# liortalker/MindTheEdge

Measured on NVIDIA B200. Metric: edge_loss_fwd_bwd_throughput, higher is better.
Workload: dtype f32

## Files before the change

### mindtheedge_b200/csrc/common.cuh

```cuda
#pragma once
#include <cuda_runtime.h>
#include <stdint.h>
#include <stdlib.h>

#include <mutex>
#include <utility>
#include <vector>

#include "../../include/mte.h"

#define MTE_FULL_MASK 0xffffffffu

#define MTE_RETURN_IF_CUDA_ERROR()                        \
    do {                                                  \
        cudaError_t e__ = cudaGetLastError();             \
        if (e__ != cudaSuccess) return (int)e__;          \
    } while (0)

namespace mte {

struct DevInfo {
    int sms;
    int smemOptin;
};
inline int current_device() {
    int d = 0;
    cudaGetDevice(&d);
    return d;
}
inline DevInfo dev_info() {
    constexpr int kMaxDev = 64;
    static DevInfo cache[kMaxDev];
    static bool have[kMaxDev];
    static std::mutex mu;
    const int d = current_device();
    std::lock_guard<std::mutex> lock(mu);
    if (d >= 0 && d < kMaxDev && have[d]) return cache[d];
    DevInfo v{148, 232448};
    cudaDeviceGetAttribute(&v.sms, cudaDevAttrMultiProcessorCount, d);
    cudaDeviceGetAttribute(&v.smemOptin, cudaDevAttrMaxSharedMemoryPerBlockOptin, d);
    if (v.sms < 1) v.sms = 1;
    if (d >= 0 && d < kMaxDev) { cache[d] = v; have[d] = true; }
    return v;
}
inline int num_sms() { return dev_info().sms; }

inline cudaError_t opt_in_smem(const void *func, int bytes) {
    static std::mutex mu;
    static std::vector<std::pair<const void *, long long>> done;
    const int d = current_device();
    std::lock_guard<std::mutex> lock(mu);
    for (auto &e : done)
        if (e.first == func && (int)(e.second >> 32) == d) {
            if ((int)(e.second & 0xffffffffLL) >= bytes) return cudaSuccess;
            const cudaError_t r = cudaFuncSetAttribute(func, cudaFuncAttributeMaxDynamicSharedMemorySize, bytes);
            if (r == cudaSuccess) e.second = ((long long)d << 32) | (unsigned)bytes;
            return r;
        }
    const cudaError_t r = cudaFuncSetAttribute(func, cudaFuncAttributeMaxDynamicSharedMemorySize, bytes);
    if (r == cudaSuccess) done.emplace_back(func, ((long long)d << 32) | (unsigned)bytes);
    return r;
}

#ifdef MTE_DEBUG_KNOBS
inline const char *debug_knob(const char *name) { return getenv(name); }
#else
inline const char *debug_knob(const char *) { return nullptr; }
#endif

struct WsHeader {
    unsigned int ticket[16];
    unsigned int flag[16];
    unsigned int pad[32];
};
static_assert(sizeof(WsHeader) == 256, "workspace header layout");
constexpr size_t kWsAccumOffset = 4096;
constexpr int kWsMaxLossImages = (MTE_WS_HEADER_BYTES - 4096) / 64;

__host__ __device__ inline size_t align_up(size_t v, size_t a) { return (v + a - 1) / a * a; }
__host__ __device__ inline int ceil_div(int a, int b) { return (a + b - 1) / b; }

__device__ __forceinline__ float warp_sum(float v) {
#pragma unroll
    for (int o = 16; o > 0; o >>= 1) v += __shfl_xor_sync(MTE_FULL_MASK, v, o);
    return v;
}
__device__ __forceinline__ double warp_sum(double v) {
#pragma unroll
    for (int o = 16; o > 0; o >>= 1) v += __shfl_xor_sync(MTE_FULL_MASK, v, o);
    return v;
}
__device__ __forceinline__ unsigned warp_or(unsigned v) {
#pragma unroll
    for (int o = 16; o > 0; o >>= 1) v |= __shfl_xor_sync(MTE_FULL_MASK, v, o);
    return v;
}

__device__ __forceinline__ float4 ld_stream4(const float *p) { return __ldcs(reinterpret_cast<const float4 *>(p)); }
__device__ __forceinline__ float4 ld_cached4(const float *p) { return __ldg(reinterpret_cast<const float4 *>(p)); }
__device__ __forceinline__ void st_stream4(float *p, float4 v) { __stcs(reinterpret_cast<float4 *>(p), v); }

inline bool aligned16(const void *p) { return (reinterpret_cast<uintptr_t>(p) & 15u) == 0; }

namespace canny {
int run_level_hysteresis(const unsigned char *cl, unsigned char *E, int N, int H, int W, int T, void *scratch,
                         cudaStream_t st);
size_t hysteresis_scratch_bytes(int N, int H, int W);
}

}
```

### mindtheedge_b200/csrc/edge_loss_fused.cu

```cuda
#include <string.h>

#include "edge_loss_kernels.cuh"

namespace mte {
namespace loss {

#ifndef MTE_FUSED_D
#define MTE_FUSED_D 3
#endif
constexpr int kFusedD = MTE_FUSED_D;
#ifndef MTE_FUSED_SEGCOST
#define MTE_FUSED_SEGCOST 2
#endif
constexpr int kSegCostFused = MTE_FUSED_SEGCOST;
#ifndef MTE_FUSED_REGS
#define MTE_FUSED_REGS 120
#endif
#ifndef MTE_FUSED_P1ROWS
#define MTE_FUSED_P1ROWS 16
#endif
constexpr int kP1Rows = MTE_FUSED_P1ROWS;
__host__ __device__ constexpr int fused_smem_bytes() { return kRWarps * kFusedD * 3 * 512; }

__device__ __forceinline__ unsigned ld_acquire_u32(const unsigned *p) {
    unsigned v;
    asm volatile("ld.acquire.gpu.global.u32 %0, [%1];" : "=r"(v) : "l"(p) : "memory");
    return v;
}

__device__ __forceinline__ void grid_barrier(unsigned *ctr, unsigned nCtas) {
    __syncthreads();
    if (threadIdx.x == 0) {
        __threadfence();
        atomicAdd(ctr, 1u);
#ifdef MTE_FUSED_NOSLEEP
        while (ld_acquire_u32(ctr) < nCtas) {}
#else
        while (ld_acquire_u32(ctr) < nCtas) __nanosleep(20);
#endif
        __threadfence();
    }
    __syncthreads();
}

#ifdef MTE_FUSED_TRACE
__device__ __forceinline__ unsigned long long gtime() {
    unsigned long long t;
    asm volatile("mov.u64 %0, %globaltimer;" : "=l"(t));
    return t;
}
#define MTE_TRACE(slot, isMin)                                                                                   \
    do {                                                                                                         \
        __syncthreads();                                                                                         \
        if (threadIdx.x == 0) {                                                                                  \
            const unsigned long long t_ = gtime();                                                               \
            atomicMax(reinterpret_cast<unsigned long long *>(F.barrier) + 128 + (slot), (isMin) ? ~t_ : t_); \
        }                                                                                                        \
    } while (0)
#else
#define MTE_TRACE(slot, isMin) do {} while (0)
#endif

struct FusedP {
    LossP L;
    const float *expectG;
    unsigned *barrier;
};

struct Seg {
    int si, img, strip, row0, nrows;
};
__device__ __forceinline__ bool next_segment(const LossP &P, int &u0, int u1, Seg &s) {
    int si = 0;
#pragma unroll
    for (int k = 1; k < MTE_MAX_SCALES; k++)
        if (k < P.nScales && u0 >= P.s[k].unitBase) si = k;
    const ScaleP &S = P.s[si];
    const int local = u0 - S.unitBase;
    const int HV = ((S.H + 1) >> 1) + kSegCostFused;
    const int t = local / HV;
    const int r = local - t * HV;
    const int take = min(HV - r, u1 - u0);
    s.row0 = 2 * max(r - kSegCostFused, 0);
    s.nrows = min(2 * max(r + take - kSegCostFused, 0), S.H) - s.row0;
    u0 += take;
    s.si = si;
    s.img = t / S.strips;
    s.strip = t - s.img * S.strips;
    return s.nrows > 0;
}

__device__ __forceinline__ void red_add4(float *p, float4 v) {
    asm volatile("red.global.add.v4.f32 [%0], {%1, %2, %3, %4};" ::"l"(p), "f"(v.x), "f"(v.y), "f"(v.z), "f"(v.w) : "memory");
}

__device__ __forceinline__ float2 f2(float s) { return make_float2(s, s); }
__device__ __forceinline__ float2 f2add(float2 a, float2 b) { return __fadd2_rn(a, b); }
__device__ __forceinline__ float2 f2mul(float2 a, float2 b) { return __fmul2_rn(a, b); }
__device__ __forceinline__ float2 f2fma(float2 a, float2 b, float2 c) { return __ffma2_rn(a, b, c); }
__device__ __forceinline__ float2 f2sub(float2 a, float2 b) { return __ffma2_rn(b, f2(-1.f), a); }
__device__ __forceinline__ float2 rcp_rn_normal2(float2 d) {
    float2 r = make_float2(rcp_approx(d.x), rcp_approx(d.y));
    const float2 nd = f2mul(d, f2(-1.f));
    float2 e = f2fma(nd, r, f2(1.f));
    r = f2fma(r, e, r);
    e = f2fma(nd, r, f2(1.f));
    return f2fma(r, e, r);
}

struct PRow2 {
    float2 c[2], s3[2], d[2];
};
__device__ __forceinline__ void prep_row2(PRow2 &R, const float2 (&x)[2]) {
    const float l = __shfl_up_sync(MTE_FULL_MASK, x[1].y, 1);
    const float r = __shfl_down_sync(MTE_FULL_MASK, x[0].x, 1);
    R.c[0] = x[0];
    R.c[1] = x[1];
    R.s3[0] = make_float2((l + x[0].x) + x[0].y, (x[0].x + x[0].y) + x[1].x);
    R.s3[1] = make_float2((x[0].y + x[1].x) + x[1].y, (x[1].x + x[1].y) + r);
    R.d[0] = make_float2(x[0].y - l, x[1].x - x[0].x);
    R.d[1] = make_float2(x[1].y - x[0].y, r - x[1].x);
}

__device__ __forceinline__ void fused_prologue(const ScaleP &S, const Seg &sg, int lane, unsigned char *ring,
                                               float2 (&xa)[2], float2 (&xc)[2]) {
    constexpr int D = kFusedD;
    constexpr unsigned PLB = 512, SLB = 3 * PLB;
    const int H = S.H, row0 = sg.row0, niter = sg.nrows;
    const unsigned W = (unsigned)S.W;
    const int col0 = (sg.strip * kHaloLanes + lane - 1) * 4;
    const bool colOk = col0 >= 0 && col0 < (int)W;
    const size_t lo = (size_t)sg.img * H * W + (colOk ? col0 : 0);
    const float *xP = S.x + lo, *eP = S.e + lo, *nP = S.n + lo;
    const unsigned ringS = (unsigned)__cvta_generic_to_shared(ring + lane * 16);
    auto load_plain = [&](float2 (&x)[2], int row) {
        x[0] = make_float2(0.f, 0.f);
        x[1] = make_float2(0.f, 0.f);
        if (colOk && row >= 0 && row < H) {
            const float4 t = ld_cached4(elem_addr(xP, (unsigned)row * W));
            x[0] = make_float2(t.x, t.y);
            x[1] = make_float2(t.z, t.w);
        }
    };
    load_plain(xa, row0 - 1);
    load_plain(xc, row0);
#pragma unroll
    for (int k = 0; k < D; k++) {
        if (k < niter) {
            const int rx = row0 + 1 + k;
            cp_async_vec<4>(ringS + k * SLB, elem_addr(xP, (unsigned)min(rx, H - 1) * W), colOk && rx < H);
            const unsigned ro = (unsigned)(row0 + k) * W;
            cp_async_vec<4>(ringS + k * SLB + PLB, elem_addr(eP, ro), colOk);
            cp_async_vec<4>(ringS + k * SLB + 2 * PLB, elem_addr(nP, ro), colOk);
        }
        cp_async_commit();
    }
}

template <bool INV, bool SIG>
__device__ __forceinline__ void fused_segment(const LossP &P, const ScaleP &S, const Seg &sg, int lane,
                                              unsigned char *ring, const float4 *sLut, float cp, float cn,
                                              float2 (&la)[2], float &poison, float2 (&xa)[2], float2 (&xc)[2]) {
    constexpr int D = kFusedD;
    constexpr unsigned PLB = 512, SLB = 3 * PLB;
    constexpr float kFill = INV ? 3.0e38f : 0.f;
    const int H = S.H, row0 = sg.row0, nrows = sg.nrows;
    const unsigned W = (unsigned)S.W;
    const int col0 = (sg.strip * kHaloLanes + lane - 1) * 4;
    const bool colOk = col0 >= 0 && col0 < (int)W;
    const bool writer = colOk && lane >= 1 && lane <= kHaloLanes;
    const size_t lo = (size_t)sg.img * H * W + (colOk ? col0 : 0);
    const float *xP = S.x + lo, *eP = S.e + lo, *nP = S.n + lo;
    float *gP = S.g + lo, *dP = S.dx + lo;
    const bool writeG = writer && S.g != nullptr;
    const float2 mT = f2(-P.T), cp2 = f2(cp), cn2 = f2(cn), eps2 = f2(kEps), one2 = f2(1.f), m1 = f2(-1.f);
    unsigned char *slot0 = ring + lane * 16;
    const unsigned ringS = (unsigned)__cvta_generic_to_shared(slot0);

    auto issue = [&](unsigned so, int j) {
        const int rx = row0 + 1 + j;
        cp_async_vec<4>(ringS + so, elem_addr(xP, (unsigned)min(rx, H - 1) * W), colOk && rx < H);
        const unsigned ro = (unsigned)(row0 + j) * W;
        cp_async_vec<4>(ringS + so + PLB, elem_addr(eP, ro), colOk);
        cp_async_vec<4>(ringS + so + 2 * PLB, elem_addr(nP, ro), colOk);
    };
    auto fix_row = [&](float2 (&x)[2], int row) {
        if (INV) {
            const bool ok = colOk && row >= 0 && row < H;
#pragma unroll
            for (int h = 0; h < 2; h++) {
                const float2 v = make_float2(fmax_nan(ok ? x[h].x : kFill, 1e-6f), fmax_nan(ok ? x[h].y : kFill, 1e-6f));
                x[h] = rcp_rn_normal2(v);
            }
        }
        const float2 t = f2fma(x[0], f2(0.f), f2mul(x[1], f2(0.f)));
        poison += t.x + t.y;
    };
    auto lds2 = [&](float2 (&x)[2], const unsigned char *p) {
        const float4 t = *reinterpret_cast<const float4 *>(p);
        x[0] = make_float2(t.x, t.y);
        x[1] = make_float2(t.z, t.w);
    };

    const int niter = nrows;
    PRow2 win[3];
    fix_row(xa, row0 - 1);
    fix_row(xc, row0);
    prep_row2(win[0], xa);
    prep_row2(win[1], xc);
    float oacc[3][4];
#pragma unroll
    for (int o = 0; o < 3; o++)
#pragma unroll
        for (int v = 0; v < 4; v++) oacc[o][v] = 0.f;
    auto emit = [&](const float (&acc)[4], const PRow2 &dep, int row, bool shared) {
        float out[4];
#pragma unroll
        for (int v = 0; v < 4; v++) {
            float d = acc[v];
            if (INV) {
                const float dp = (v & 1) ? dep.c[v >> 1].y : dep.c[v >> 1].x;
                d = (dp < 1e6f) ? -d * dp * dp : 0.f;
            }
            out[v] = d;
        }
        if (writer) {
            float *o = elem_addr(dP, (unsigned)row * W);
            if (shared) red_add4(o, make_float4(out[0], out[1], out[2], out[3]));
            else st_stream4(o, make_float4(out[0], out[1], out[2], out[3]));
        }
    };

    unsigned so = 0;
#pragma unroll 1
    for (int jj = 0; jj < niter; jj += 3) {
#pragma unroll
        for (int u = 0; u < 3; u++) {
            const int j = jj + u;
            if (j < niter) {
                cp_async_wait<D - 1>();
                float2 xn[2], e[2], th[2];
                lds2(xn, slot0 + so);
                lds2(e, slot0 + so + PLB);
                lds2(th, slot0 + so + 2 * PLB);
                if (j + D < niter) issue(so, j + D);
                cp_async_commit();
                so = (so + SLB == D * SLB) ? 0u : so + SLB;
                const int r = row0 + j;
                PRow2 &dn = win[(u + 2) % 3];
                fix_row(xn, r + 1);
                prep_row2(dn, xn);
                const PRow2 &up = win[u % 3];
                const PRow2 &mid = win[(u + 1) % 3];
                float g[4];
                float2 X[4], Z[4];
#pragma unroll
                for (int h = 0; h < 2; h++) {
                    const float2 Pv = f2sub(dn.s3[h], up.s3[h]);
                    const float2 Dm = mid.d[h];
                    const float2 Rh = f2add(f2add(up.d[h], Dm), dn.d[h]);
                    const float2 dv = f2sub(dn.c[h], up.c[h]);
                    float c0, c1;
                    unsigned cd0, cd1;
                    pick_directional(th[h].x, Pv.x, Rh.x, Dm.x, dv.x, c0, cd0);
                    pick_directional(th[h].y, Pv.y, Rh.y, Dm.y, dv.y, c1, cd1);
                    const float2 gg = make_float2(fabsf(c0), fabsf(c1));
                    g[2 * h] = gg.x;
                    g[2 * h + 1] = gg.y;
                    float2 p = gg;
                    if (SIG) {
                        const float2 nz = f2sub(f2(P.T), gg);
                        p = rcp_rn_normal2(f2add(make_float2(expf(nz.x), expf(nz.y)), one2));
                    }
                    const float2 q = f2fma(p, m1, one2);
                    const float2 pe = f2add(p, eps2), qe = f2add(q, eps2);
                    const float2 ee = e[h], ne = f2fma(ee, m1, one2);
                    la[0] = f2fma(ee, make_float2(lg2_approx(pe.x), lg2_approx(pe.y)), la[0]);
                    la[1] = f2fma(ne, make_float2(lg2_approx(qe.x), lg2_approx(qe.y)), la[1]);
                    float2 d = f2mul(f2mul(cp2, ee), make_float2(rcp_approx(pe.x), rcp_approx(pe.y)));
                    d = f2fma(f2mul(cn2, ne), make_float2(rcp_approx(qe.x), rcp_approx(qe.y)), d);
                    if (SIG) d = f2mul(f2mul(d, p), q);
                    const float d0 = (colOk && gg.x != 0.f) ? d.x : 0.f, d1 = (colOk && gg.y != 0.f) ? d.y : 0.f;
                    const float4 k0 = sLut[cd0 & 15u], k1 = sLut[cd1 & 15u];
                    X[2 * h] = f2mul(f2(d0), make_float2(k0.x, k0.y));
                    Z[2 * h] = f2mul(f2(d0), make_float2(k0.z, k0.w));
                    X[2 * h + 1] = f2mul(f2(d1), make_float2(k1.x, k1.y));
                    Z[2 * h + 1] = f2mul(f2(d1), make_float2(k1.z, k1.w));
                }
                if (writeG) st_stream4(elem_addr(gP, (unsigned)r * W), make_float4(g[0], g[1], g[2], g[3]));
                const float2 Xl = make_float2(__shfl_up_sync(MTE_FULL_MASK, X[3].x, 1), __shfl_up_sync(MTE_FULL_MASK, X[3].y, 1));
                const float2 Xr = make_float2(__shfl_down_sync(MTE_FULL_MASK, X[0].x, 1), __shfl_down_sync(MTE_FULL_MASK, X[0].y, 1));
                const float C2l = __shfl_up_sync(MTE_FULL_MASK, Z[3].y, 1), C2r = __shfl_down_sync(MTE_FULL_MASK, Z[0].y, 1);
#pragma unroll
                for (int v = 0; v < 4; v++) {
                    const float2 xl = v == 0 ? Xl : X[(v + 3) % 4], xr = v == 3 ? Xr : X[(v + 1) % 4];
                    const float c2_l = v == 0 ? C2l : Z[(v + 3) % 4].y, c2_r = v == 3 ? C2r : Z[(v + 1) % 4].y;
                    const float2 U = f2add(xl, make_float2(xr.x, -xr.y));
                    const float SA = U.x + Z[v].x, DC = U.y;
                    oacc[u][v] = SA + DC;
                    oacc[(u + 2) % 3][v] += c2_l - c2_r;
                    oacc[(u + 1) % 3][v] -= SA - DC;
                }
                if (r >= 1) emit(oacc[(u + 1) % 3], up, r - 1, j < 2);
                if (j == niter - 1) {
                    emit(oacc[(u + 2) % 3], mid, r, true);
                    if (r + 1 < H) emit(oacc[u], dn, r + 1, true);
                }
            }
        }
    }
    cp_async_wait<0>();
    if (!writer) {
        la[0] = f2(0.f);
        la[1] = f2(0.f);
    }
}

template <bool INV, bool SIG>
__global__ void __maxnreg__(MTE_FUSED_REGS) edge_loss_fused_kernel(const __grid_constant__ FusedP F) {
    extern __shared__ __align__(16) unsigned char fusedRing[];
    __shared__ float4 sLut[16];
    __shared__ double sLoss[MTE_MAX_SCALES];
    __shared__ int sLast;
    const LossP &P = F.L;
    if (threadIdx.x < 16) {
        const int di = threadIdx.x & 3, sgn_ = threadIdx.x >> 2;
        const float sgn = sgn_ == 1 ? 1.f : (sgn_ == 2 ? -1.f : 0.f);
        const float a = (di == 2 || di == 3) ? 1.f : (di == 1 ? -1.f : 0.f);
        const float c = (di == 2) ? 0.f : 1.f;
        const float bb = (di & 1) ? 1.f : 2.f;
        sLut[threadIdx.x] = make_float4(sgn * a, sgn * c, sgn * a * bb, sgn * c * bb);
    }
    const int lane = threadIdx.x & 31, warp = threadIdx.x >> 5;
    const int nWarps = gridDim.x * kRWarps;
    const int gw = blockIdx.x * kRWarps + warp;
    unsigned char *ring = fusedRing + warp * (fused_smem_bytes() / kRWarps);
    const int uBeg = (int)((long long)P.totalUnits * gw / nWarps);
    const int uEnd = (int)((long long)P.totalUnits * (gw + 1) / nWarps);
    pdl_launch_dependents();
    MTE_TRACE(0, true);
    MTE_TRACE(1, false);

#ifndef MTE_FUSED_TIMING_NO_PHASE1
    {
        int u0 = uBeg;
        while (u0 < uEnd) {
            Seg sg;
            if (!next_segment(P, u0, uEnd, sg)) continue;
            const ScaleP &S = P.s[sg.si];
            const unsigned W = (unsigned)S.W;
            const int col0 = (sg.strip * kHaloLanes + lane - 1) * 4;
            const bool writer = col0 >= 0 && col0 < (int)W && lane >= 1 && lane <= kHaloLanes;
            const float *eP = S.e + (size_t)sg.img * S.H * W + (writer ? col0 : 0);
            if (writer) {
                float *dP = S.dx + (size_t)sg.img * S.H * W + col0;
                const float4 z = make_float4(0.f, 0.f, 0.f, 0.f);
                *reinterpret_cast<float4 *>(elem_addr(dP, (unsigned)sg.row0 * W)) = z;
                *reinterpret_cast<float4 *>(elem_addr(dP, (unsigned)(sg.row0 + sg.nrows - 1) * W)) = z;
            }
            float s0 = 0.f, s1 = 0.f;
#pragma unroll 1
            for (int j0 = 0; j0 < sg.nrows; j0 += kP1Rows) {
                float4 t[kP1Rows];
#pragma unroll
                for (int k = 0; k < kP1Rows; k++) {
                    t[k] = make_float4(0.f, 0.f, 0.f, 0.f);
                    if (writer && j0 + k < sg.nrows)
                        t[k] = *reinterpret_cast<const float4 *>(elem_addr(eP, (unsigned)(sg.row0 + j0 + k) * W));
                }
#pragma unroll
                for (int k = 0; k < kP1Rows; k += 2) {
                    s0 += (t[k].x + t[k].y) + (t[k].z + t[k].w);
                    s1 += (t[k + 1].x + t[k + 1].y) + (t[k + 1].z + t[k + 1].w);
                }
            }
            const float v = warp_sum(s0 + s1);
            unsigned long long *acc = P.accum + (size_t)(S.imgBase + sg.img) * kAcc;
            if (lane == 0) {
                atomicAdd(acc + A_WP, (unsigned long long)__double2ll_rn((double)v * kFix));
                if (!isfinite(v)) atomicOr(acc + A_FLAGS, (unsigned long long)F_NONFINITE);
            }
        }
    }
    int u0 = uBeg;
    Seg sg;
    bool have = false;
    while (u0 < uEnd && !have) have = next_segment(P, u0, uEnd, sg);
    float2 xa[2], xc[2];
    if (have) fused_prologue(P.s[sg.si], sg, lane, ring, xa, xc);
    MTE_TRACE(2, true);
    MTE_TRACE(3, false);
    grid_barrier(F.barrier, gridDim.x);
    MTE_TRACE(4, false);
#else
    __syncthreads();
    int u0 = uBeg;
    Seg sg;
    bool have = false;
    while (u0 < uEnd && !have) have = next_segment(P, u0, uEnd, sg);
    float2 xa[2], xc[2];
    if (have) fused_prologue(P.s[sg.si], sg, lane, ring, xa, xc);
#endif

    while (have) {
        const ScaleP &S = P.s[sg.si];
        const double npix = (double)S.H * (double)S.W;
        float alpha;
        {
            const double wp = (double)(long long)__ldcg(P.accum + (size_t)(S.imgBase + sg.img) * kAcc + A_WP) / kFix;
            const double wn = npix - wp;
            alpha = (float)(wn / (wp + wn));
            if (wn == 0.0) {
                double wnSum = 0.0;
                for (int b = 0; b < S.B; b++)
                    wnSum += npix - (double)(long long)__ldcg(P.accum + (size_t)(S.imgBase + b) * kAcc + A_WP) / kFix;
                if (wnSum == 0.0) alpha = 1.0f;
            }
        }
        float G = F.expectG ? (__ldg(F.expectG) * S.scaleWeight + __ldg(F.expectG + 1 + sg.si)) : S.scaleWeight;
        if (G == 0.f) G = 1.f;
        const float coef = (float)((double)P.weight / (npix * (double)S.B)) * G;
        const float cp = -coef * P.p2n * alpha, cn = coef * (1.0f - alpha);
        float2 la[2] = {make_float2(0.f, 0.f), make_float2(0.f, 0.f)};
        float poison = 0.f;
        fused_segment<INV, SIG>(P, S, sg, lane, ring, sLut, cp, cn, la, poison, xa, xc);
        bool bad = __any_sync(MTE_FULL_MASK, !(poison == 0.f));
        unsigned long long *acc = P.accum + (size_t)(S.imgBase + sg.img) * kAcc;
        const float vp = warp_sum(la[0].x + la[0].y), vn = warp_sum(la[1].x + la[1].y);
        bad = bad || !isfinite(vp) || !isfinite(vn);
        if (lane == 0) {
            atomicAdd(acc + A_SPU, (unsigned long long)__double2ll_rn((double)vp * kFix));
            atomicAdd(acc + A_SNU, (unsigned long long)__double2ll_rn((double)vn * kFix));
            if (bad) atomicOr(acc + A_FLAGS, (unsigned long long)F_NONFINITE);
        }
        have = false;
        while (u0 < uEnd && !have) have = next_segment(P, u0, uEnd, sg);
        if (have) fused_prologue(P.s[sg.si], sg, lane, ring, xa, xc);
    }
    MTE_TRACE(5, true);
    MTE_TRACE(6, false);
    __syncthreads();
    if (threadIdx.x == 0) {
        __threadfence();
        sLast = atomicAdd(P.ticket + 1, 1u) == gridDim.x - 1u;
        __threadfence();
    }
    __syncthreads();
    if (sLast) {
        finalize_loss<false>(P, sLoss);
        __syncthreads();
        if (threadIdx.x == 0) {
            double total = 0.0;
            for (int k = 0; k < P.nScales; k++) {
                total += (double)P.s[k].scaleWeight * sLoss[k];
                float G = F.expectG ? (F.expectG[0] * P.s[k].scaleWeight + F.expectG[1 + k]) : P.s[k].scaleWeight;
                if (G == 0.f) G = 1.f;
                P.ctx[P.totalImages + 2 * MTE_MAX_SCALES + k] = G;
            }
            reinterpret_cast<unsigned *>(P.ctx + P.totalImages + 3 * MTE_MAX_SCALES)[0] = 0u;
            P.lossOut[0] = (float)total;
            P.ticket[0] = 0u;
            P.ticket[1] = 0u;
            *F.barrier = 0u;
        }
        MTE_TRACE(7, false);
    }
}

__global__ void __launch_bounds__(128) edge_loss_rescale_kernel(const __grid_constant__ LossP P, const float *gradLoss,
                                                                float *ctx, float *expectedOut) {
    pdl_wait();
    float *cur = ctx + P.totalImages + 2 * MTE_MAX_SCALES;
    unsigned *done = reinterpret_cast<unsigned *>(ctx + P.totalImages + 3 * MTE_MAX_SCALES);
    bool any = false;
    for (int k = 0; k < P.nScales; k++) any = any || (gradLoss[0] * P.s[k].scaleWeight + gradLoss[1 + k] != cur[k]);
    if (!any) {
        if (expectedOut && blockIdx.x == 0 && threadIdx.x <= P.nScales) expectedOut[threadIdx.x] = gradLoss[threadIdx.x];
        return;
    }
    for (int k = 0; k < P.nScales; k++) {
        const ScaleP &S = P.s[k];
        const float G = gradLoss[0] * S.scaleWeight + gradLoss[1 + k];
        const float c = cur[k];
        if (G == c) continue;
        const float f = G / c;
        const size_t n4 = (size_t)S.B * S.H * S.W / 4;
        float4 *d = reinterpret_cast<float4 *>(S.dx);
        for (size_t i = (size_t)blockIdx.x * blockDim.x + threadIdx.x; i < n4; i += (size_t)gridDim.x * blockDim.x) {
            float4 v = d[i];
            v.x *= f; v.y *= f; v.z *= f; v.w *= f;
            d[i] = v;
        }
    }
    __syncthreads();
    if (threadIdx.x == 0) {
        __threadfence();
        if (atomicAdd(done, 1u) == gridDim.x - 1u) {
            for (int k = 0; k < P.nScales; k++) cur[k] = gradLoss[0] * P.s[k].scaleWeight + gradLoss[1 + k];
            if (expectedOut)
                for (int k = 0; k < 1 + P.nScales; k++) expectedOut[k] = gradLoss[k];
            __threadfence();
            *done = 0u;
        }
    }
}

template <bool INV, bool SIG>
static int launch_fused_one(const FusedP &F, int grid, cudaStream_t st) {
    constexpr int smem = fused_smem_bytes();
    const void *fn = (const void *)edge_loss_fused_kernel<INV, SIG>;
    if (opt_in_smem(fn, smem) != cudaSuccess) return (int)cudaGetLastError();
    int perSm = 0;
    cudaOccupancyMaxActiveBlocksPerMultiprocessor(&perSm, edge_loss_fused_kernel<INV, SIG>, kRThreads, smem);
    if (perSm < 1) return MTE_ERR_ARG;
    const int maxGrid = perSm * num_sms();
    if (grid > maxGrid) grid = maxGrid;
    cudaLaunchConfig_t cfg = {};
    cfg.gridDim = dim3((unsigned)grid);
    cfg.blockDim = dim3((unsigned)kRThreads);
    cfg.dynamicSmemBytes = (size_t)smem;
    cfg.stream = st;
    cudaLaunchAttribute at[1];
    at[0].id = cudaLaunchAttributeCooperative;
    at[0].val.cooperative = 1;
    cfg.attrs = at;
    cfg.numAttrs = 1;
    const cudaError_t e = cudaLaunchKernelEx(&cfg, edge_loss_fused_kernel<INV, SIG>, F);
    return e == cudaSuccess ? MTE_OK : (int)e;
}

int launch_fused(const FusedP &F, int grid, bool inv, bool sig, cudaStream_t st) {
    if (inv) return sig ? launch_fused_one<true, true>(F, grid, st) : launch_fused_one<true, false>(F, grid, st);
    return sig ? launch_fused_one<false, true>(F, grid, st) : launch_fused_one<false, false>(F, grid, st);
}

}
}

using namespace mte;
using namespace mte::loss;

static bool fused_supported(const mte_loss_scale_t *sc, int n, const mte_loss_attrs_t *at) {
    if (!sc || !at || n < 1 || n > MTE_MAX_SCALES) return false;
    if (!at->is_grad) return false;
    for (int i = 0; i < n; i++) {
        const mte_loss_scale_t &s = sc[i];
        if (!s.pred || !s.edge || !s.normal || s.mask) return false;
        if (s.h != s.H || s.w != s.W || s.B < 1 || s.H < 1 || s.W < 4 || (s.W % 4)) return false;
        const void *ptrs[] = {s.pred, s.edge, s.normal, s.grad_map, s.grad_pred};
        for (const void *p : ptrs)
            if (!aligned16(p)) return false;
    }
    return true;
}

extern "C" int mte_edge_loss_fused_supported(const mte_loss_scale_t *sc, int n, const mte_loss_attrs_t *at) {
    return fused_supported(sc, n, at) ? 1 : 0;
}

extern "C" int mte_edge_loss_fwd_grad(const mte_loss_scale_t *sc, int n, const mte_loss_attrs_t *at,
                                      const float *expected_grad_loss, float *loss_out, void *ctx, void *ws,
                                      size_t ws_bytes, mte_stream_t stream) {
    if (!sc || !at || !loss_out || !ctx || !ws) return MTE_ERR_NULL;
    if (!fused_supported(sc, n, at)) return MTE_ERR_ARG;
    for (int i = 0; i < n; i++)
        if (!sc[i].grad_pred) return MTE_ERR_NULL;
    if (ws_bytes < MTE_WS_HEADER_BYTES) return MTE_ERR_WORKSPACE;
    FusedP F;
    memset(&F, 0, sizeof(F));
    LossP &P = F.L;
    int img = 0;
    long long unitBase = 0;
    for (int i = 0; i < n; i++) {
        ScaleP &S = P.s[i];
        S.B = sc[i].B; S.H = sc[i].H; S.W = sc[i].W;
        S.x = sc[i].pred; S.e = sc[i].edge; S.n = sc[i].normal; S.m = nullptr;
        S.g = sc[i].grad_map; S.dx = sc[i].grad_pred; S.stash = nullptr;
        S.strips = ceil_div(S.W, kHaloLanes * 4);
        S.imgBase = img;
        S.unitBase = (int)unitBase;
        unitBase += (long long)S.strips * (((S.H + 1) >> 1) + kSegCostFused) * S.B;
        S.scaleWeight = sc[i].scale_weight;
        img += S.B;
    }
    if (unitBase > 0x7fffffffLL || img > kWsMaxLossImages) return MTE_ERR_SHAPE;
    P.nScales = n; P.totalImages = img; P.totalUnits = (int)unitBase;
    P.T = at->sigmoid_thresh; P.weight = at->weight; P.p2n = at->pos_to_neg;
    char *w = static_cast<char *>(ws);
    WsHeader *hdr = reinterpret_cast<WsHeader *>(w);
    P.accum = reinterpret_cast<unsigned long long *>(w + kWsAccumOffset);
    P.ticket = hdr->ticket;
    P.lossOut = loss_out;
    P.ctx = static_cast<float *>(ctx);
    F.expectG = expected_grad_loss;
    F.barrier = hdr->ticket + 2;
    int grid = num_sms();
    const int minUnits = 2;
    if ((long long)grid * kRWarps * minUnits > unitBase) grid = (int)((unitBase + kRWarps * minUnits - 1) / (kRWarps * minUnits));
    if (grid < 1) grid = 1;
    return launch_fused(F, grid, at->pred_is_inverse != 0, at->is_sigmoid != 0, reinterpret_cast<cudaStream_t>(stream));
}

extern "C" int mte_edge_loss_grad_rescale(const mte_loss_scale_t *sc, int n, const float *grad_loss, void *ctx,
                                          float *expected_out, mte_stream_t stream) {
    if (!sc || !grad_loss || !ctx) return MTE_ERR_NULL;
    if (n < 1 || n > MTE_MAX_SCALES) return MTE_ERR_ARG;
    LossP P;
    memset(&P, 0, sizeof(P));
    int img = 0;
    for (int i = 0; i < n; i++) {
        if (!sc[i].grad_pred) return MTE_ERR_NULL;
        if (!aligned16(sc[i].grad_pred) || (sc[i].W % 4)) return MTE_ERR_ALIGN;
        P.s[i].B = sc[i].B; P.s[i].H = sc[i].H; P.s[i].W = sc[i].W;
        P.s[i].dx = sc[i].grad_pred;
        P.s[i].scaleWeight = sc[i].scale_weight;
        img += sc[i].B;
    }
    P.nScales = n; P.totalImages = img;
    cudaLaunchConfig_t cfg = {};
    cfg.gridDim = dim3((unsigned)num_sms() * 2u);
    cfg.blockDim = dim3(128u);
    cfg.stream = reinterpret_cast<cudaStream_t>(stream);
    cudaLaunchAttribute at[1];
    at[0].id = cudaLaunchAttributeProgrammaticStreamSerialization;
    at[0].val.programmaticStreamSerializationAllowed = 1;
    cfg.attrs = at;
    cfg.numAttrs = 1;
    const cudaError_t e = cudaLaunchKernelEx(&cfg, edge_loss_rescale_kernel, P, grad_loss, static_cast<float *>(ctx), expected_out);
    return e == cudaSuccess ? MTE_OK : (int)e;
}
```

Before: 132,600.

## Split fused loss phase-1 sums into PDL-chained kernel, drop grid barrier

The per-image edge sums that used to be computed in a first phase of the cooperative fused kernel, followed by a software grid barrier, now run in a separate kernel. That kernel streams rows through a cp.async ring buffer in shared memory. The fused kernel is launched with programmatic dependent launch so it can run its prologue while the sums kernel finishes, then calls pdl_wait before the main loop. The aim is to remove the grid-wide spin barrier and cooperative launch and to overlap the prologue with the reduction. It also sets a max-shared carveout and halves the rescale kernel grid, at the cost of one extra kernel launch.

```diff
diff --git a/mindtheedge_b200/csrc/common.cuh b/mindtheedge_b200/csrc/common.cuh
--- a/mindtheedge_b200/csrc/common.cuh
+++ b/mindtheedge_b200/csrc/common.cuh
@@ -45,7 +45,7 @@
 }
 inline int num_sms() { return dev_info().sms; }
 
-inline cudaError_t opt_in_smem(const void *func, int bytes) {
+inline cudaError_t opt_in_smem(const void *func, int bytes, int carveout = -1) {
     static std::mutex mu;
     static std::vector<std::pair<const void *, long long>> done;
     const int d = current_device();
@@ -57,7 +57,9 @@
             if (r == cudaSuccess) e.second = ((long long)d << 32) | (unsigned)bytes;
             return r;
         }
-    const cudaError_t r = cudaFuncSetAttribute(func, cudaFuncAttributeMaxDynamicSharedMemorySize, bytes);
+    cudaError_t r = cudaFuncSetAttribute(func, cudaFuncAttributeMaxDynamicSharedMemorySize, bytes);
+    if (r == cudaSuccess && carveout >= 0)
+        r = cudaFuncSetAttribute(func, cudaFuncAttributePreferredSharedMemoryCarveout, carveout);
     if (r == cudaSuccess) done.emplace_back(func, ((long long)d << 32) | (unsigned)bytes);
     return r;
 }
diff --git a/mindtheedge_b200/csrc/edge_loss_fused.cu b/mindtheedge_b200/csrc/edge_loss_fused.cu
--- a/mindtheedge_b200/csrc/edge_loss_fused.cu
+++ b/mindtheedge_b200/csrc/edge_loss_fused.cu
@@ -16,32 +16,19 @@
 #ifndef MTE_FUSED_REGS
 #define MTE_FUSED_REGS 120
 #endif
-#ifndef MTE_FUSED_P1ROWS
-#define MTE_FUSED_P1ROWS 16
-#endif
-constexpr int kP1Rows = MTE_FUSED_P1ROWS;
 __host__ __device__ constexpr int fused_smem_bytes() { return kRWarps * kFusedD * 3 * 512; }
 
-__device__ __forceinline__ unsigned ld_acquire_u32(const unsigned *p) {
-    unsigned v;
-    asm volatile("ld.acquire.gpu.global.u32 %0, [%1];" : "=r"(v) : "l"(p) : "memory");
-    return v;
-}
-
-__device__ __forceinline__ void grid_barrier(unsigned *ctr, unsigned nCtas) {
-    __syncthreads();
-    if (threadIdx.x == 0) {
-        __threadfence();
-        atomicAdd(ctr, 1u);
-#ifdef MTE_FUSED_NOSLEEP
-        while (ld_acquire_u32(ctr) < nCtas) {}
-#else
-        while (ld_acquire_u32(ctr) < nCtas) __nanosleep(20);
-#endif
-        __threadfence();
-    }
-    __syncthreads();
-}
+#ifndef MTE_SUMS_WARPS
+#define MTE_SUMS_WARPS 16
+#endif
+#ifndef MTE_SUMS_ROWS
+#define MTE_SUMS_ROWS 4
+#endif
+constexpr int kSumWarps = MTE_SUMS_WARPS, kSumThreads = kSumWarps * 32;
+constexpr int kSumRows = MTE_SUMS_ROWS, kSumStages = 4;
+constexpr unsigned kSumRowBytes = 32 * 16;
+constexpr unsigned kSumStageBytes = kSumRows * kSumRowBytes;
+__host__ __device__ constexpr int sums_smem_bytes() { return kSumWarps * kSumStages * (int)kSumStageBytes; }
 
 #ifdef MTE_FUSED_TRACE
 __device__ __forceinline__ unsigned long long gtime() {
@@ -49,22 +36,22 @@
     asm volatile("mov.u64 %0, %globaltimer;" : "=l"(t));
     return t;
 }
-#define MTE_TRACE(slot, isMin)                                                                                   \
-    do {                                                                                                         \
-        __syncthreads();                                                                                         \
-        if (threadIdx.x == 0) {                                                                                  \
-            const unsigned long long t_ = gtime();                                                               \
-            atomicMax(reinterpret_cast<unsigned long long *>(F.barrier) + 128 + (slot), (isMin) ? ~t_ : t_); \
-        }                                                                                                        \
+__device__ __forceinline__ void trace_put(unsigned *base, int slot, bool isMin, unsigned long long t) {
+    atomicMax(reinterpret_cast<unsigned long long *>(base) + 128 + slot, isMin ? ~t : t);
+}
+#define MTE_TRACE(base, slot, isMin)                                   \
+    do {                                                                 \
+        __syncthreads();                                                 \
+        if (threadIdx.x == 0) trace_put((base), (slot), (isMin), gtime()); \
     } while (0)
 #else
-#define MTE_TRACE(slot, isMin) do {} while (0)
+#define MTE_TRACE(base, slot, isMin) do {} while (0)
 #endif
 
 struct FusedP {
     LossP L;
     const float *expectG;
-    unsigned *barrier;
+    unsigned *trace;
 };
 
 struct Seg {
@@ -92,6 +79,109 @@
 
 __device__ __forceinline__ void red_add4(float *p, float4 v) {
     asm volatile("red.global.add.v4.f32 [%0], {%1, %2, %3, %4};" ::"l"(p), "f"(v.x), "f"(v.y), "f"(v.z), "f"(v.w) : "memory");
+}
+
+__device__ __forceinline__ float4 lds_f4(unsigned addr) {
+    float4 v;
+    asm volatile("ld.shared.v4.f32 {%0, %1, %2, %3}, [%4];" : "=f"(v.x), "=f"(v.y), "=f"(v.z), "=f"(v.w) : "r"(addr) : "memory");
+    return v;
+}
+
+__global__ void __launch_bounds__(kSumThreads, 65536 / (kSumThreads * 32)) edge_loss_sums_kernel(const __grid_constant__ FusedP F, int nItems) {
+    extern __shared__ __align__(16) unsigned char sumRing[];
+    __shared__ unsigned sDesc[kSumWarps][kSumStages];
+    const LossP &P = F.L;
+    const int lane = threadIdx.x & 31, warp = threadIdx.x >> 5;
+    const unsigned ringS = (unsigned)__cvta_generic_to_shared(sumRing + warp * kSumStages * kSumStageBytes) + lane * 16;
+    pdl_wait();
+    pdl_launch_dependents();
+    MTE_TRACE(F.trace, 0, true);
+    MTE_TRACE(F.trace, 1, false);
+
+    const int nW = gridDim.x * kSumWarps, gw = blockIdx.x * kSumWarps + warp;
+    int it = (int)((long long)nItems * gw / nW);
+    const int itEnd = (int)((long long)nItems * (gw + 1) / nW);
+    int u0 = 0, u1 = 0, siStrip = 0, img = 0, row = 0, rowEnd = 0;
+    auto produce = [&](int slot) -> bool {
+        while (row >= rowEnd) {
+            if (u0 < u1) {
+                Seg sg;
+                if (next_segment(P, u0, u1, sg)) {
+                    siStrip = sg.si | sg.strip << 2;
+                    img = sg.img;
+                    row = sg.row0;
+                    rowEnd = sg.row0 + sg.nrows;
+                    const ScaleP &S = P.s[sg.si];
+                    const int col0 = (sg.strip * kHaloLanes + lane - 1) * 4;
+                    if (lane >= 1 && lane <= kHaloLanes && col0 < S.W) {
+                        float *dP = S.dx + (size_t)img * S.H * S.W + col0;
+                        const float4 z = make_float4(0.f, 0.f, 0.f, 0.f);
+                        *reinterpret_cast<float4 *>(elem_addr(dP, (unsigned)row * S.W)) = z;
+                        *reinterpret_cast<float4 *>(elem_addr(dP, (unsigned)(rowEnd - 1) * S.W)) = z;
+                    }
+                }
+                continue;
+            }
+            if (it >= itEnd) return false;
+            u0 = (int)((long long)P.totalUnits * it / nItems);
+            u1 = (int)((long long)P.totalUnits * (it + 1) / nItems);
+            it++;
+        }
+        const ScaleP &S = P.s[siStrip & 3];
+        const int strip = siStrip >> 2;
+        const int n = min(kSumRows, rowEnd - row);
+        const int col0 = (strip * kHaloLanes + lane - 1) * 4;
+        const bool ok = lane >= 1 && lane <= kHaloLanes && col0 < S.W;
+        if (lane == 0) sDesc[warp][slot] = (unsigned)(S.imgBase + img) | (unsigned)n << 12 | (row + n == rowEnd ? 1u << 24 : 0u);
+        const float *eP = S.e + (size_t)img * S.H * S.W + (ok ? col0 : 0);
+#pragma unroll
+        for (int k = 0; k < kSumRows; k++)
+            if (k < n) cp_async_vec<4>(ringS + slot * kSumStageBytes + k * kSumRowBytes, elem_addr(eP, (unsigned)(row + k) * S.W), ok);
+        cp_async_commit();
+        row += n;
+        return true;
+    };
+
+    bool more = true;
+    int c = 0, p = 0;
+    for (int k = 0; k < kSumStages && more; k++) {
+        more = produce(k);
+        if (more) p++;
+    }
+    float s0 = 0.f, s1 = 0.f;
+    while (c < p) {
+        const int slot = c & (kSumStages - 1);
+        if (p - c == kSumStages) cp_async_wait<kSumStages - 1>();
+        else cp_async_wait<0>();
+        __syncwarp();
+        const unsigned d = sDesc[warp][slot];
+        const int n = (d >> 12) & 31;
+#pragma unroll
+        for (int k = 0; k < kSumRows; k++) {
+            float4 a = make_float4(0.f, 0.f, 0.f, 0.f);
+            if (k < n) a = lds_f4(ringS + slot * kSumStageBytes + k * kSumRowBytes);
+            if (k & 1) s1 += (a.x + a.y) + (a.z + a.w);
+            else s0 += (a.x + a.y) + (a.z + a.w);
+        }
+        if (d >> 24) {
+            const float v = warp_sum(s0 + s1);
+            if (lane == 0) {
+                unsigned long long *acc = P.accum + (size_t)(d & 0xfffu) * kAcc;
+                atomicAdd(acc + A_WP, (unsigned long long)__double2ll_rn((double)v * kFix));
+                if (!isfinite(v)) atomicOr(acc + A_FLAGS, (unsigned long long)F_NONFINITE);
+            }
+            s0 = 0.f;
+            s1 = 0.f;
+        }
+        __syncwarp();
+        c++;
+        if (more) {
+            more = produce(p & (kSumStages - 1));
+            if (more) p++;
+        }
+    }
+    MTE_TRACE(F.trace, 2, true);
+    MTE_TRACE(F.trace, 3, false);
 }
 
 __device__ __forceinline__ float2 f2(float s) { return make_float2(s, s); }
@@ -331,6 +421,9 @@
         const float bb = (di & 1) ? 1.f : 2.f;
         sLut[threadIdx.x] = make_float4(sgn * a, sgn * c, sgn * a * bb, sgn * c * bb);
     }
+#ifdef MTE_FUSED_TRACE
+    const unsigned long long tStart = gtime();
+#endif
     const int lane = threadIdx.x & 31, warp = threadIdx.x >> 5;
     const int nWarps = gridDim.x * kRWarps;
     const int gw = blockIdx.x * kRWarps + warp;
@@ -338,69 +431,23 @@
     const int uBeg = (int)((long long)P.totalUnits * gw / nWarps);
     const int uEnd = (int)((long long)P.totalUnits * (gw + 1) / nWarps);
     pdl_launch_dependents();
-    MTE_TRACE(0, true);
-    MTE_TRACE(1, false);
-
-#ifndef MTE_FUSED_TIMING_NO_PHASE1
-    {
-        int u0 = uBeg;
-        while (u0 < uEnd) {
-            Seg sg;
-            if (!next_segment(P, u0, uEnd, sg)) continue;
-            const ScaleP &S = P.s[sg.si];
-            const unsigned W = (unsigned)S.W;
-            const int col0 = (sg.strip * kHaloLanes + lane - 1) * 4;
-            const bool writer = col0 >= 0 && col0 < (int)W && lane >= 1 && lane <= kHaloLanes;
-            const float *eP = S.e + (size_t)sg.img * S.H * W + (writer ? col0 : 0);
-            if (writer) {
-                float *dP = S.dx + (size_t)sg.img * S.H * W + col0;
-                const float4 z = make_float4(0.f, 0.f, 0.f, 0.f);
-                *reinterpret_cast<float4 *>(elem_addr(dP, (unsigned)sg.row0 * W)) = z;
-                *reinterpret_cast<float4 *>(elem_addr(dP, (unsigned)(sg.row0 + sg.nrows - 1) * W)) = z;
-            }
-            float s0 = 0.f, s1 = 0.f;
-#pragma unroll 1
-            for (int j0 = 0; j0 < sg.nrows; j0 += kP1Rows) {
-                float4 t[kP1Rows];
-#pragma unroll
-                for (int k = 0; k < kP1Rows; k++) {
-                    t[k] = make_float4(0.f, 0.f, 0.f, 0.f);
-                    if (writer && j0 + k < sg.nrows)
-                        t[k] = *reinterpret_cast<const float4 *>(elem_addr(eP, (unsigned)(sg.row0 + j0 + k) * W));
-                }
-#pragma unroll
-                for (int k = 0; k < kP1Rows; k += 2) {
-                    s0 += (t[k].x + t[k].y) + (t[k].z + t[k].w);
-                    s1 += (t[k + 1].x + t[k + 1].y) + (t[k + 1].z + t[k + 1].w);
-                }
-            }
-            const float v = warp_sum(s0 + s1);
-            unsigned long long *acc = P.accum + (size_t)(S.imgBase + sg.img) * kAcc;
-            if (lane == 0) {
-                atomicAdd(acc + A_WP, (unsigned long long)__double2ll_rn((double)v * kFix));
-                if (!isfinite(v)) atomicOr(acc + A_FLAGS, (unsigned long long)F_NONFINITE);
-            }
-        }
-    }
+
     int u0 = uBeg;
     Seg sg;
     bool have = false;
     while (u0 < uEnd && !have) have = next_segment(P, u0, uEnd, sg);
     float2 xa[2], xc[2];
     if (have) fused_prologue(P.s[sg.si], sg, lane, ring, xa, xc);
-    MTE_TRACE(2, true);
-    MTE_TRACE(3, false);
-    grid_barrier(F.barrier, gridDim.x);
-    MTE_TRACE(4, false);
-#else
+    pdl_wait();
     __syncthreads();
-    int u0 = uBeg;
-    Seg sg;
-    bool have = false;
-    while (u0 < uEnd && !have) have = next_segment(P, u0, uEnd, sg);
-    float2 xa[2], xc[2];
-    if (have) fused_prologue(P.s[sg.si], sg, lane, ring, xa, xc);
-#endif
+#ifdef MTE_FUSED_TRACE
+    if (threadIdx.x == 0) {
+        trace_put(F.trace, 4, true, tStart);
+        trace_put(F.trace, 5, false, tStart);
+    }
+#endif
+    MTE_TRACE(F.trace, 6, true);
+    MTE_TRACE(F.trace, 7, false);
 
     while (have) {
         const ScaleP &S = P.s[sg.si];
@@ -437,8 +484,8 @@
         while (u0 < uEnd && !have) have = next_segment(P, u0, uEnd, sg);
         if (have) fused_prologue(P.s[sg.si], sg, lane, ring, xa, xc);
     }
-    MTE_TRACE(5, true);
-    MTE_TRACE(6, false);
+    MTE_TRACE(F.trace, 8, true);
+    MTE_TRACE(F.trace, 9, false);
     __syncthreads();
     if (threadIdx.x == 0) {
         __threadfence();
@@ -461,14 +508,14 @@
             P.lossOut[0] = (float)total;
             P.ticket[0] = 0u;
             P.ticket[1] = 0u;
-            *F.barrier = 0u;
-        }
-        MTE_TRACE(7, false);
-    }
-}
-
-__global__ void __launch_bounds__(128) edge_loss_rescale_kernel(const __grid_constant__ LossP P, const float *gradLoss,
-                                                                float *ctx, float *expectedOut) {
+        }
+        MTE_TRACE(F.trace, 10, false);
+    }
+}
+
+__global__ void __launch_bounds__(128, 16) edge_loss_rescale_kernel(const __grid_constant__ LossP P, const float *gradLoss,
+                                                                    float *ctx, float *expectedOut) {
+    pdl_launch_dependents();
     pdl_wait();
     float *cur = ctx + P.totalImages + 2 * MTE_MAX_SCALES;
     unsigned *done = reinterpret_cast<unsigned *>(ctx + P.totalImages + 3 * MTE_MAX_SCALES);
@@ -505,27 +552,33 @@
     }
 }
 
+template <typename... Args>
+static cudaError_t launch_dependent(void (*kernel)(Args...), int grid, int block, int smem, cudaStream_t st,
+                                    const Args &...args) {
+    cudaLaunchConfig_t cfg = {};
+    cfg.gridDim = dim3((unsigned)grid);
+    cfg.blockDim = dim3((unsigned)block);
+    cfg.dynamicSmemBytes = (size_t)smem;
+    cfg.stream = st;
+    cudaLaunchAttribute at[1];
+    at[0].id = cudaLaunchAttributeProgrammaticStreamSerialization;
+    at[0].val.programmaticStreamSerializationAllowed = 1;
+    cfg.attrs = at;
+    cfg.numAttrs = 1;
+    return cudaLaunchKernelEx(&cfg, kernel, args...);
+}
+
 template <bool INV, bool SIG>
 static int launch_fused_one(const FusedP &F, int grid, cudaStream_t st) {
     constexpr int smem = fused_smem_bytes();
     const void *fn = (const void *)edge_loss_fused_kernel<INV, SIG>;
-    if (opt_in_smem(fn, smem) != cudaSuccess) return (int)cudaGetLastError();
-    int perSm = 0;
-    cudaOccupancyMaxActiveBlocksPerMultiprocessor(&perSm, edge_loss_fused_kernel<INV, SIG>, kRThreads, smem);
-    if (perSm < 1) return MTE_ERR_ARG;
-    const int maxGrid = perSm * num_sms();
-    if (grid > maxGrid) grid = maxGrid;
-    cudaLaunchConfig_t cfg = {};
-    cfg.gridDim = dim3((unsigned)grid);
-    cfg.blockDim = dim3((unsigned)kRThreads);
-    cfg.dynamicSmemBytes = (size_t)smem;
-    cfg.stream = st;
-    cudaLaunchAttribute at[1];
-    at[0].id = cudaLaunchAttributeCooperative;
-    at[0].val.cooperative = 1;
-    cfg.attrs = at;
-    cfg.numAttrs = 1;
-    const cudaError_t e = cudaLaunchKernelEx(&cfg, edge_loss_fused_kernel<INV, SIG>, F);
+    if (opt_in_smem(fn, smem, cudaSharedmemCarveoutMaxShared) != cudaSuccess) return (int)cudaGetLastError();
+    if (opt_in_smem((const void *)edge_loss_sums_kernel, sums_smem_bytes(), cudaSharedmemCarveoutMaxShared) != cudaSuccess)
+        return (int)cudaGetLastError();
+    const int nItems = grid * kRWarps;
+    const int sumGrid = min(num_sms(), ceil_div(nItems, kSumWarps));
+    cudaError_t e = launch_dependent(edge_loss_sums_kernel, sumGrid, kSumThreads, sums_smem_bytes(), st, F, nItems);
+    if (e == cudaSuccess) e = launch_dependent(edge_loss_fused_kernel<INV, SIG>, grid, kRThreads, smem, st, F);
     return e == cudaSuccess ? MTE_OK : (int)e;
 }
 
@@ -593,7 +646,7 @@
     P.lossOut = loss_out;
     P.ctx = static_cast<float *>(ctx);
     F.expectG = expected_grad_loss;
-    F.barrier = hdr->ticket + 2;
+    F.trace = hdr->ticket + 2;
     int grid = num_sms();
     const int minUnits = 2;
     if ((long long)grid * kRWarps * minUnits > unitBase) grid = (int)((unitBase + kRWarps * minUnits - 1) / (kRWarps * minUnits));
@@ -618,7 +671,7 @@
     }
     P.nScales = n; P.totalImages = img;
     cudaLaunchConfig_t cfg = {};
-    cfg.gridDim = dim3((unsigned)num_sms() * 2u);
+    cfg.gridDim = dim3((unsigned)num_sms());
     cfg.blockDim = dim3(128u);
     cfg.stream = reinterpret_cast<cudaStream_t>(stream);
     cudaLaunchAttribute at[1];
```

Result: faster. 134,300, median of 6 (+1.2%).

## Split grid barrier into arrive/wait and use release/acquire atomics

Applied to the files above, without the earlier changes.

The grid barrier becomes a split arrive/wait pair: each CTA signals arrival with a release reduction before running the segment prologue and waits only afterward, so prologue work overlaps barrier latency. Spin loops use relaxed loads followed by one acquire load, and the final ticket uses an acq_rel atomic instead of fences around a plain atomicAdd. The rescale kernel is also unrolled to four float4 loads per thread with half the grid size. The memory-ordering changes are subtle and could expose races if the prologue reads data written before other CTAs arrive.

```diff
diff --git a/mindtheedge_b200/csrc/edge_loss_fused.cu b/mindtheedge_b200/csrc/edge_loss_fused.cu
--- a/mindtheedge_b200/csrc/edge_loss_fused.cu
+++ b/mindtheedge_b200/csrc/edge_loss_fused.cu
@@ -27,18 +27,29 @@
     asm volatile("ld.acquire.gpu.global.u32 %0, [%1];" : "=r"(v) : "l"(p) : "memory");
     return v;
 }
-
-__device__ __forceinline__ void grid_barrier(unsigned *ctr, unsigned nCtas) {
+__device__ __forceinline__ unsigned ld_relaxed_u32(const unsigned *p) {
+    unsigned v;
+    asm volatile("ld.relaxed.gpu.global.u32 %0, [%1];" : "=r"(v) : "l"(p) : "memory");
+    return v;
+}
+__device__ __forceinline__ unsigned atom_add_acq_rel_u32(unsigned *p, unsigned v) {
+    unsigned old;
+    asm volatile("atom.acq_rel.gpu.global.add.u32 %0, [%1], %2;" : "=r"(old) : "l"(p), "r"(v) : "memory");
+    return old;
+}
+
+__device__ __forceinline__ void grid_arrive(unsigned *ctr) {
     __syncthreads();
+    if (threadIdx.x == 0) asm volatile("red.release.gpu.global.add.u32 [%0], 1;" ::"l"(ctr) : "memory");
+}
+__device__ __forceinline__ void grid_wait(const unsigned *ctr, unsigned nCtas) {
     if (threadIdx.x == 0) {
-        __threadfence();
-        atomicAdd(ctr, 1u);
 #ifdef MTE_FUSED_NOSLEEP
-        while (ld_acquire_u32(ctr) < nCtas) {}
+        while (ld_relaxed_u32(ctr) < nCtas) {}
 #else
-        while (ld_acquire_u32(ctr) < nCtas) __nanosleep(20);
+        while (ld_relaxed_u32(ctr) < nCtas) __nanosleep(20);
 #endif
-        __threadfence();
+        (void)ld_acquire_u32(ctr);
     }
     __syncthreads();
 }
@@ -382,15 +393,17 @@
             }
         }
     }
+    MTE_TRACE(2, true);
+    MTE_TRACE(3, false);
+    grid_arrive(F.barrier);
     int u0 = uBeg;
     Seg sg;
     bool have = false;
     while (u0 < uEnd && !have) have = next_segment(P, u0, uEnd, sg);
     float2 xa[2], xc[2];
     if (have) fused_prologue(P.s[sg.si], sg, lane, ring, xa, xc);
-    MTE_TRACE(2, true);
-    MTE_TRACE(3, false);
-    grid_barrier(F.barrier, gridDim.x);
+    grid_wait(F.barrier, gridDim.x);
+    MTE_TRACE(8, true);
     MTE_TRACE(4, false);
 #else
     __syncthreads();
@@ -440,13 +453,10 @@
     MTE_TRACE(5, true);
     MTE_TRACE(6, false);
     __syncthreads();
-    if (threadIdx.x == 0) {
-        __threadfence();
-        sLast = atomicAdd(P.ticket + 1, 1u) == gridDim.x - 1u;
-        __threadfence();
-    }
+    if (threadIdx.x == 0) sLast = atom_add_acq_rel_u32(P.ticket + 1, 1u) == gridDim.x - 1u;
     __syncthreads();
     if (sLast) {
+        MTE_TRACE(9, false);
         finalize_loss<false>(P, sLoss);
         __syncthreads();
         if (threadIdx.x == 0) {
@@ -467,8 +477,10 @@
     }
 }
 
-__global__ void __launch_bounds__(128) edge_loss_rescale_kernel(const __grid_constant__ LossP P, const float *gradLoss,
-                                                                float *ctx, float *expectedOut) {
+constexpr int kRescaleThreads = 128;
+constexpr int kRescaleVec = 4;
+__global__ void __launch_bounds__(kRescaleThreads, 65536 / (kRescaleThreads * 32))
+edge_loss_rescale_kernel(const __grid_constant__ LossP P, const float *gradLoss, float *ctx, float *expectedOut) {
     pdl_wait();
     float *cur = ctx + P.totalImages + 2 * MTE_MAX_SCALES;
     unsigned *done = reinterpret_cast<unsigned *>(ctx + P.totalImages + 3 * MTE_MAX_SCALES);
@@ -486,10 +498,18 @@
         const float f = G / c;
         const size_t n4 = (size_t)S.B * S.H * S.W / 4;
         float4 *d = reinterpret_cast<float4 *>(S.dx);
-        for (size_t i = (size_t)blockIdx.x * blockDim.x + threadIdx.x; i < n4; i += (size_t)gridDim.x * blockDim.x) {
-            float4 v = d[i];
-            v.x *= f; v.y *= f; v.z *= f; v.w *= f;
-            d[i] = v;
+        const size_t step = (size_t)gridDim.x * kRescaleThreads * kRescaleVec;
+        for (size_t i0 = (size_t)blockIdx.x * kRescaleThreads * kRescaleVec + threadIdx.x; i0 < n4; i0 += step) {
+            float4 v[kRescaleVec];
+#pragma unroll
+            for (int u = 0; u < kRescaleVec; u++)
+                if (i0 + u * kRescaleThreads < n4) v[u] = d[i0 + u * kRescaleThreads];
+#pragma unroll
+            for (int u = 0; u < kRescaleVec; u++)
+                if (i0 + u * kRescaleThreads < n4) {
+                    v[u].x *= f; v[u].y *= f; v[u].z *= f; v[u].w *= f;
+                    d[i0 + u * kRescaleThreads] = v[u];
+                }
         }
     }
     __syncthreads();
@@ -618,8 +638,8 @@
     }
     P.nScales = n; P.totalImages = img;
     cudaLaunchConfig_t cfg = {};
-    cfg.gridDim = dim3((unsigned)num_sms() * 2u);
-    cfg.blockDim = dim3(128u);
+    cfg.gridDim = dim3((unsigned)num_sms());
+    cfg.blockDim = dim3((unsigned)kRescaleThreads);
     cfg.stream = reinterpret_cast<cudaStream_t>(stream);
     cudaLaunchAttribute at[1];
     at[0].id = cudaLaunchAttributeProgrammaticStreamSerialization;
```

After: 134,300 before, 138,400 after, median of 6. 3.1% higher.
